# pacargile/ThePayne

Hardware: AMD Instinct MI355X
Metric: likelihood-evals/sec (4k-pixel ANN, 512 live points) (higher is better)
Workload: dtype f32; 1 GPU; C2: single star per GPU, 4096-pixel 2x300 YST1 ANN, 3600 observed pixels, batch of 512 candidate vectors per step (dynesty live points); batch=512, npix=4096, nobs=3600, stars=1, kernel_variant=0, parallelism=1 star per GPU, no data-path collective, products=2 x fp16 parts, 3 products, fp32 accumulator

## Files before the change

include/payne_hip.h:

```cpp
#ifndef PAYNE_HIP_H
#define PAYNE_HIP_H

#ifdef __cplusplus
extern "C" {
#endif

#define PAYNE_ABI_VERSION 2

#define PAYNE_OK 0
#define PAYNE_E_INVALID (-1)
#define PAYNE_E_UNSUPPORTED (-2)
#define PAYNE_E_HIP (-3)
#define PAYNE_E_BATCH (-4)
#define PAYNE_E_SIGMA (-5)

#define PAYNE_ACT_NONE 0
#define PAYNE_ACT_LRELU 1
#define PAYNE_ACT_SIGMOID 2

#define PAYNE_MAX_LAYERS 8
#define PAYNE_MAX_LABELS 5
#define PAYNE_MAX_POLY 12

typedef struct payne_layer {
// ... 44 lines not shown
} payne_opts;

#define PAYNE_V_OUT_GENERIC 1u
#define PAYNE_V_POST_GENERIC 2u
#define PAYNE_V_TW_GLOBAL 4u
#define PAYNE_V_POST_FULL 8u
#define PAYNE_V_NO_PREP 16u
#define PAYNE_V_SELECT_MEDIAN 64u
#define PAYNE_V_NO_WALK_TAIL 512u
#define PAYNE_V_OUT_BK64 1024u
#define PAYNE_V_OUT_ROLLED 2048u
#define PAYNE_V_OUT_F32 4096u
#define PAYNE_V_SED_OWN_LAUNCH 8192u
#define PAYNE_V_OUT_SMALL_TILES 16384u
#define PAYNE_V_BIG_WORKSPACE 65536u
#define PAYNE_V_NO_WALK_SPEC 131072u
#define PAYNE_V_ROWS_PIXEL 262144u
#define PAYNE_V_OUT_PLANES 524288u
#define PAYNE_V_OUT_BF16X3 1048576u
#define PAYNE_V_HID_F32 2097152u
#define PAYNE_V_HID_CHAIN 4194304u
#define PAYNE_V_HID_WAVES4 8388608u
#define PAYNE_V_OUT_WHOLE_TILE 16777216u
#define PAYNE_V_LSF_GLOBAL 128u

typedef struct payne_ctx payne_ctx;

int payne_version(void);

int payne_ctx_create(const payne_model_desc* model, const payne_obs_desc* obs,
                     const payne_phot_desc* phot, const payne_opts* opts, int device,
                     payne_ctx** out);

int payne_ctx_set_obs(payne_ctx* ctx, const payne_obs_desc* obs);

int payne_ctx_set_continuum(payne_ctx* ctx, const payne_model_desc* cont);

int payne_ctx_set_lsf(payne_ctx* ctx, const double* lsf, int n);
int payne_ctx_set_lsf_on(payne_ctx* ctx, const double* lsf_wave, const double* lsf, int n);

void payne_ctx_destroy(payne_ctx* ctx);

const char* payne_last_error(const payne_ctx* ctx);

int payne_theta_cols(const payne_ctx* ctx);

// ... 161 lines not shown
```

thepayne_amd/_lib.py:

```python
import ctypes as C
import os

HERE = os.path.dirname(os.path.abspath(__file__))
LIB_PATH = os.path.join(HERE, "libpayne_hip.so")

PAYNE_MAX_LAYERS = 8
PAYNE_MAX_POLY = 12
ACT_NONE, ACT_LRELU, ACT_SIGMOID = 0, 1, 2
F_FWHM_R = 1
SMOOTH_VEL_DIRECT, SMOOTH_WAVE_DIRECT, SMOOTH_LSF_DIRECT, SMOOTH_WAVE_FFT, SMOOTH_INTERP = range(5)
ABI_VERSION = 2
E_INVALID, E_UNSUPPORTED, E_HIP, E_BATCH, E_SIGMA = -1, -2, -3, -4, -5
V_OUT_GENERIC, V_POST_GENERIC, V_TW_GLOBAL, V_POST_FULL, V_NO_PREP, V_SELECT_MEDIAN, V_LSF_GLOBAL, V_NO_WALK_TAIL, V_OUT_BK64, V_OUT_ROLLED, V_OUT_F32, V_SED_OWN_LAUNCH, V_BIG_WORKSPACE = 1, 2, 4, 8, 16, 64, 128, 512, 1024, 2048, 4096, 8192, 65536
V_OUT_SMALL_TILES = 16384
V_NO_WALK_SPEC = 131072
V_ROWS_PIXEL = 262144
V_OUT_PLANES = 524288
V_OUT_BF16X3 = 1048576
V_HID_F32 = 2097152
V_HID_CHAIN = 4194304
V_HID_WAVES4 = 8388608
V_OUT_WHOLE_TILE = 16777216

SYMBOLS = ["payne_version", "payne_ctx_create", "payne_ctx_set_obs", "payne_ctx_set_continuum", "payne_ctx_set_lsf", "payne_ctx_set_lsf_on", "payne_ctx_destroy", "payne_last_error",
           "payne_theta_cols", "payne_lnlike_batch", "payne_predict_batch", "payne_smooth_batch", "payne_smooth_direct", "payne_sed_batch", "payne_bc_batch", "payne_kernel_name", "payne_last_kernel", "payne_activation_batch",
           "payne_profile", "payne_profile_read",
           "payne_sampler_create", "payne_sampler_destroy", "payne_prior_transform_batch", "payne_lnprob_u_batch",
           "payne_rwalk_batch", "payne_rwalk_begin", "payne_rwalk_begin_ell", "payne_rwalk_step", "payne_sampler_counters", "payne_ns_rwalk_queue", "payne_ns_rwalk_queue_begin", "payne_ns_rwalk_queue_end", "payne_ns_rwalk_queue_turn", "payne_ns_consume", "payne_ns_peek", "payne_ns_bound", "payne_format_rows",
           "payne_ns_queue_dev_init", "payne_ns_queue_dev_launch", "payne_ns_queue_dev_collect"]

PAYNE_MAX_DIM, PAYNE_MAX_FIXED = 24, 16
PRIOR_UNIFORM, PRIOR_GAUSSIAN, PRIOR_TGAUSSIAN, PRIOR_EXP, PRIOR_TEXP, PRIOR_LOGUNIFORM, PRIOR_TABLE = range(7)

_dp = C.POINTER(C.c_double)


class Layer(C.Structure):
    _fields_ = [("w", C.c_void_p), ("b", C.c_void_p), ("n_in", C.c_int), ("n_out", C.c_int), ("act", C.c_int)]


class ModelDesc(C.Structure):
    _fields_ = [("n_layers", C.c_int), ("layers", Layer * PAYNE_MAX_LAYERS), ("n_labels", C.c_int),
                ("xmin", _dp), ("xmax", _dp), ("npix", C.c_int), ("wavelength", _dp), ("resolution", C.c_double)]


# ... 171 lines not shown
```

thepayne_amd/csrc/k_post_full_a.hip:

```cpp
#define PAYNE_TU_POST_FULL_A
#include <hip/hip_runtime.h>

#include "../../include/payne_hip.h"
#include "post_seq.hpp"

using namespace payne;
#include "post_kernels.hpp"
PAYNE_POST_FULL_A_LIST(PAYNE_POST_DEFINE)
```

thepayne_amd/csrc/k_post_lean.hip:

```cpp
#define PAYNE_TU_POST_LEAN
#include <hip/hip_runtime.h>

#include "../../include/payne_hip.h"
#include "post_seq.hpp"

using namespace payne;
#include "post_kernels.hpp"
PAYNE_POST_LEAN_LIST(PAYNE_POST_DEFINE)
```

thepayne_amd/csrc/payne_hip.hip:

```cpp
#include <hip/hip_runtime.h>

#include <chrono>
#include <cstdio>
#include <cstdlib>
#include <cstring>
#include <string>
#include <thread>
#include <vector>

#include "../../include/payne_hip.h"
#include "host_tables.hpp"
#include "post_seq.hpp"
#include "ns_core.hpp"

using namespace payne;

#include "dense_kernels.hpp"

#include "post_kernels.hpp"

#include "sed_kernel.hpp"
#include "select.hpp"

__global__ void payne_photonly_kernel(const double* mags, const double* obs, const double* err, int F, int B, double* lnl) {
// ... 467 lines not shown
      }
      c->big_tiled = true;
      c->big_chip = T.n1 == kChipN1 && c->H.geo && !(opts->variant & PAYNE_V_BIG_WORKSPACE);
      if (c->big_chip) {
        he = hipFuncSetAttribute(reinterpret_cast<const void*>(payne_post_chip_kernel), hipFuncAttributeMaxDynamicSharedMemorySize,
                                 (int)kChipLdsBytes);
        if (he != hipSuccess) return bail(fail(c, PAYNE_E_HIP, std::string("hipFuncSetAttribute(chip): ") + hipGetErrorString(he)));
      }
      if (c->big_tiled) {
        he = hipFuncSetAttribute(reinterpret_cast<const void*>(payne_post_big_kernel), hipFuncAttributeMaxDynamicSharedMemorySize,
                                 (int)(2 * fft_tile_complex() * sizeof(c32)));
        if (he != hipSuccess) return bail(fail(c, PAYNE_E_HIP, std::string("hipFuncSetAttribute(big): ") + hipGetErrorString(he)));
      }
    }
    c->post_lds = (size_t)(T.n1 > 16384 ? 64 : fft_buf_floats(T.n1)) * 8 + (size_t)scratch_doubles(kPostThreads) * 8 + ((sizeof(CandState) + 15) & ~(size_t)15) + 16;
    const size_t tw_bytes = c->H.twf.size() * sizeof(c32);
    c->post_tw_lds = (c->post_lds + tw_bytes) <= 80 * 1024;
    if (opts->variant & PAYNE_V_TW_GLOBAL) c->post_tw_lds = false;
    if (c->post_tw_lds) c->post_lds += tw_bytes;
#ifdef PAYNE_STAMPS
    if (const char* e = getenv("PAYNE_DIAG_LDS")) c->post_lds = std::max(c->post_lds, (size_t)atoi(e));
#endif
    const int geom_n1 = (opts->variant & PAYNE_V_POST_GENERIC) ? 0 : T.n1;
    c->post_fn = pick_post_kernel(geom_n1, c->post_tw_lds);
    c->post_fn_lean = (opts->variant & PAYNE_V_POST_FULL) ? c->post_fn : pick_post_kernel(geom_n1, c->post_tw_lds, true);
    c->lean_available = c->post_fn_lean != c->post_fn;
    he = hipFuncSetAttribute(reinterpret_cast<const void*>(c->post_fn_lean), hipFuncAttributeMaxDynamicSharedMemorySize, (int)c->post_lds);
    if (he != hipSuccess) return bail(fail(c, PAYNE_E_HIP, std::string("hipFuncSetAttribute: ") + hipGetErrorString(he)));
    he = hipFuncSetAttribute(reinterpret_cast<const void*>(c->post_fn), hipFuncAttributeMaxDynamicSharedMemorySize, (int)c->post_lds);
    if (he != hipSuccess) return bail(fail(c, PAYNE_E_HIP, std::string("hipFuncSetAttribute: ") + hipGetErrorString(he)));
    {
      const bool fixed = geom_n1 != 0 && ((c->post_tw_lds && (T.n1 == 1024 || T.n1 == 2048 || T.n1 == 4096)) || (!c->post_tw_lds && T.n1 == 8192));
      const bool ident = T.rot_identity && T.n1 == model->npix;
      if (((fixed || c->big_chip || c->big_chip2) && ident || (fixed && !ident)) && c->w_out_p3 && c->hid_p3 && !(opts->variant & PAYNE_V_ROWS_PIXEL)) {
        const payne_layer& L = model->layers[model->n_layers - 1];
        const int K = L.n_in, Kp = c->w_out_kp, n = ident ? L.n_out : T.n1;
        std::vector<float> W((size_t)L.n_out * K), b((size_t)L.n_out), Wz, bz;
        he = hipMemcpy(W.data(), L.w, W.size() * 4, hipMemcpyDeviceToHost);
        if (he == hipSuccess) he = hipMemcpy(b.data(), L.b, b.size() * 4, hipMemcpyDeviceToHost);
        if (he != hipSuccess) return bail(fail(c, PAYNE_E_HIP, std::string("hipMemcpy(output layer): ") + hipGetErrorString(he)));
        if (ident) freq_rows(W.data(), b.data(), -(double)kBase, n, K, Wz, bz, c->big_chip ? 1 : (c->big_chip2 ? 2 : 0));
        else {
          freq_rows(W.data(), b.data(), -(double)kBase, n, K, Wz, bz, 0, c->H.rs1_idx.data(), c->H.rs1_frac.data(), L.n_out);
          c->freq_rs = true;
          if ((rc = dev_alloc(c, (size_t)1, &c->rot_flag, c->owned))) return bail(rc);
        }
        std::vector<float> Wp((size_t)n * Kp, 0.f);
        for (int i = 0; i < n; ++i) std::copy(Wz.begin() + (size_t)i * K, Wz.begin() + (size_t)(i + 1) * K, Wp.begin() + (size_t)i * Kp);
// ... 607 lines not shown
  a.prep = c->prep_valid ? c->prep : nullptr;
  const bool lean = stage < 0 && !out && a.prep && !c->big_ws;
  if (tail && lean && c->lean_available) {
    a.tail = tail->dev; a.tail_step = tail->step; a.tail_propose = tail->propose; tail->done = true;
    a.tail_spec = (c->spec_launched && tail->propose && tail->spec) ? 1 : 0;
  }
  {
    ProfScope ps(c, s, 1);
    if (c->big_ws && c->big_chip) {
      const int grid = B < c->big_grid ? B : c->big_grid;
      PAYNE_LAUNCH(payne_post_chip_kernel, dim3(grid), dim3(kChipThreads), kChipLdsBytes, s, c->T, a, c->big_ws, B);
    } else if (c->big_ws && c->big_chip2) {
      const int pairs = (B + 1) / 2, grid = pairs < c->big_grid ? pairs : c->big_grid;
      PAYNE_LAUNCH(payne_post_chip2_kernel, dim3(grid), dim3(kChipThreads), kChipLdsBytes, s, c->T, a, c->big_ws, B);
    } else if (c->big_ws) {
      const int grid = B < c->big_grid ? B : c->big_grid;
      const int tiled = c->big_tiled ? 1 : 0;
      const size_t lds = (tiled & 1) ? 2 * (size_t)fft_tile_complex() * sizeof(c32) : 0;
      PAYNE_LAUNCH(payne_post_big_kernel, dim3(grid), dim3(kBigThreads), lds, s, c->T, a, c->big_ws, B, tiled);
    } else {
      if (!post_lead_fits(a.ld_raw, a.ld_theta, a.n_filters)) return fail(c, PAYNE_E_INVALID, "row pitch / theta columns / filters beyond what the post kernel's packed arguments hold");
      PAYNE_LAUNCH(lean ? c->post_fn_lean : c->post_fn, dim3(B), dim3(kPostThreads), c->post_lds, s, c->T.twf, a.raw, a.prep, a.theta,
                   a.rot_flag, a.mags, post_lead_ints(a.ld_raw, a.ld_theta, a.n_filters, c->T.raw_freq), (unsigned)a.rot_seq, c->T, a);
      c->last_kernel[1] = post_kernel_label((c->opts.variant & PAYNE_V_POST_GENERIC) ? 0 : c->T.n1, c->post_tw_lds, lean && c->lean_available);
    }
  }
  hipError_t e = hipGetLastError();
  if (e != hipSuccess) return fail(c, PAYNE_E_HIP, std::string("post launch: ") + hipGetErrorString(e));
  return PAYNE_OK;
}

static int run_post_lsf(payne_ctx* c, const double* theta, int B, int stage, float* out, int ld_out, double* lnl,
                        bool with_phot, hipStream_t s) {
  const bool had = c->has_lsf;
  for (int off = 0; off < B; off += c->lsf_chunk) {
    const int nb = std::min(c->lsf_chunk, B - off);
    const double* th = theta + (size_t)off * c->ncols;
    c->has_lsf = false;
    const float* raw_all = c->raw;
    const CandState* prep_all = c->prep;
    c->raw = const_cast<float*>(raw_all) + (size_t)off * c->T.npix;
    c->prep = const_cast<CandState*>(prep_all) + off;
    int rc = run_post(c, th, nb, 1.0, 5, c->lsf_spec, c->T.npix, nullptr, false, s);
    c->raw = const_cast<float*>(raw_all); c->prep = const_cast<CandState*>(prep_all);
    c->has_lsf = had;
    if (rc) return rc;
    LsfArgs a{};
// ... 1026 lines not shown
```

thepayne_amd/csrc/post_core.hpp:

```cpp
#pragma once
#include <math.h>
#include <stdint.h>

#ifdef __HIPCC__
#define PAYNE_HD __host__ __device__ __forceinline__
#define PAYNE_HD_COLD __host__ __device__ inline __attribute__((noinline))
#else
#define PAYNE_HD inline
#define PAYNE_HD_COLD inline
#endif

namespace payne {

constexpr double kCkms = 2.998e5;
constexpr double kCDoppler = 299792.458;
constexpr double kPi = 3.141592653589793;
constexpr float kBase = 1.0f;
constexpr double kVsTabStep = 1.0 / 64.0;
constexpr double kVsTabMax = 256.0;
constexpr double kPosMagic = 1572864.0;
constexpr unsigned kPosMagicHi = 0x41380000u;
constexpr int kObsPad = 8192;
#ifndef PAYNE_POST_THREADS
#define PAYNE_POST_THREADS 512
// ... 506 lines not shown
        w[2] = ldc1(twf, OFF + P + k); w[4] = ldc1(twf, OFF + 2 * P + k);
        w[3] = cmul(w[1], w[2]); w[5] = cmul(w[1], w[4]); w[6] = cmul(w[2], w[4]); w[7] = cmul(w[3], w[4]);
      } else if constexpr (R == 4) {
        w[2] = cmul(w[1], w[1]); w[3] = cmul(w[2], w[1]);
      }
      twiddle_all<R>(u, w);
    }
    dftR<R>(u);
    const int j = fft_lay<PO, R>((i - k) * R + k);
#pragma unroll
    for (int r = 0; r < R; ++r) {
      c32 v = u[r];
      union { float f; unsigned b; } cv;
      cv.f = v.y; cv.b ^= sign; v.y = cv.f;
      if constexpr (last) {
        if (r == 0 && edge && i == 0) v.x = v.y;
        if (r == R - 1 && edge && i == NB - 1) v.y = v.x;
      }
      stc(dst, j + r * P, v);
    }
  }
}

PAYNE_HD_COLD double vsini_sb_exact(double ub) {
  double s, c;
#ifdef __HIP_DEVICE_COMPILE__
  sincos(ub, &s, &c);
#else
  s = sin(ub); c = cos(ub);
#endif
  double u2 = ub * ub;
  return j1(ub) / ub - 3.0 * c / (2.0 * u2) + 3.0 * s / (2.0 * (u2 * ub));
}
typedef float tap2 __attribute__((vector_size(8)));
struct TapPos { int i; float f; };
PAYNE_HD TapPos vsini_tab_pos(int tab_n, double vs_c64, int k, bool& far) {
  const double tm = fma((double)k, vs_c64, kPosMagic);
  const bool in = tm < kPosMagic + (double)(tab_n - 3);
  far = far || !in;
  union { double d; unsigned long long u; } cv;
  cv.d = in ? tm : kPosMagic;
  TapPos p;
  p.i = (int)((unsigned)(cv.u >> 32) & 0x7FFFFu);
  p.f = (float)(unsigned)cv.u * 2.3283064365386963e-10f;
  return p;
}
// ... 978 lines not shown
```

thepayne_amd/csrc/post_kernels.hpp:

```cpp
#pragma once
#include "select.hpp"
#include "sampler_core.hpp"
#include "post_onchip.hpp"
#include "post_onchip2.hpp"

constexpr int kStampRow = 192;
struct PostArgs {
  const double* theta; int ld_theta;
  double instr_factor;
  const float* raw; int ld_raw;
  float* out; int ld_out; int out_stage;
  double* lnl;
  const double* mags; int n_filters;
  const double* obs_mag; const double* obs_err;
  unsigned long long* stamps;
  int stamp_sparse;
  const CandState* prep;
  const WalkTail* tail; int tail_step, tail_propose;
  int tail_spec;
  const unsigned long long* rot_flag; unsigned long long rot_seq; int ld_raw_alt;
};

template <bool BUF_LDS, bool TW_LDS, int NTHR = 0>
struct DevExecT {
  static __device__ __forceinline__ int nthr_() { if constexpr (NTHR > 0) return NTHR; else return (int)blockDim.x; }
  static constexpr bool kTwLds = TW_LDS;
#ifdef __HIP_DEVICE_COMPILE__
  static __device__ __forceinline__ auto buf(c32* p) {
    if constexpr (BUF_LDS) return (PAYNE_AS_LDS f2v*)p; else return (PAYNE_AS_GLOBAL f2v*)p;
  }
  static __device__ __forceinline__ auto twid(const c32* p) {
    if constexpr (TW_LDS) return (const PAYNE_AS_LDS f2v*)p; else return (const PAYNE_AS_GLOBAL f2v*)p;
  }
  static __device__ __forceinline__ auto lds(c32* p) { return (PAYNE_AS_LDS f2v*)p; }
#else
  static c32* buf(c32* p) { return p; }
  static const c32* twid(const c32* p) { return p; }
  static c32* lds(c32* p) { return p; }
#endif
#ifdef PAYNE_STAMPS
  unsigned long long* stamps = nullptr;
  int nst = 0;
  bool sparse = false;
#endif
  template <class F>
  __device__ __forceinline__ void par(F&& f) {
// ... 11 lines not shown
#endif
  }
  __device__ __forceinline__ int nthreads() const { return nthr_(); }
  c32* tile_ = nullptr;
  __device__ __forceinline__ c32* tile() const { return tile_; }
};

__device__ __forceinline__ double sed_chi2(const double* mags, const double* obs, const double* err, int F) {
  double s = 0.0;
  for (int f = 0; f < F; ++f) { const double d = mags[f] - obs[f]; s += (d * d) / (err[f] * err[f]); }
  return s;
}

__device__ __attribute__((noinline)) static void walk_tail(const WalkTail* t, int b, int lane, double lnl, int step, int propose) {
  const WalkState W = uniform_copy(&t->w);
  rwalk_step_wave(t->sd, W, b, lane, lnl, step, 1, propose);
}

__device__ __attribute__((noinline)) static void walk_tail_spec(const WalkTail* t, int b, int lane, double lnl) {
  const WalkState W = uniform_copy(&t->w);
  rwalk_settle_spec(W, b, lane, lnl);
}

template <int LOG2N, bool TW_LDS, bool LEAN = false>
#if PAYNE_POST_THREADS > 512
#define PAYNE_POST_BOUNDS __launch_bounds__(kPostThreads) __attribute__((amdgpu_waves_per_eu(8, 8)))
#else
#define PAYNE_POST_BOUNDS __launch_bounds__(kPostThreads)
#endif
__global__ void PAYNE_POST_BOUNDS payne_post_kernel(const c32* lead_twf, const float* lead_raw, const CandState* lead_prep, const double* lead_theta, const unsigned long long* lead_rot_flag, const double* lead_mags, unsigned lead_ints, unsigned lead_rot_seq, const PostTables T_, PostArgs a_) {
  PostTables T = T_;
  T.twf = lead_twf; T.raw_freq = (int)(lead_ints >> 31);
  PostArgs a = a_;
  a.raw = lead_raw; a.prep = lead_prep; a.theta = lead_theta; a.rot_flag = lead_rot_flag; a.mags = lead_mags;
  a.ld_raw = (int)(lead_ints & 0x1ffffu); a.ld_theta = (int)((lead_ints >> 17) & 0x3fu); a.n_filters = (int)((lead_ints >> 23) & 0xffu);
  extern __shared__ __attribute__((aligned(16))) unsigned char smem[];
  const int n1 = LOG2N > 0 ? (1 << LOG2N) : T.n1;
  int raw_freq = T.raw_freq, ld_raw = a.ld_raw;
  if (a.rot_flag != nullptr && (unsigned)*a.rot_flag == lead_rot_seq) { raw_freq = 0; ld_raw = a.ld_raw_alt; }
  float* bufA = reinterpret_cast<float*>(smem);
  float* bufB = bufA + fft_buf_floats(n1);
  double* red = reinterpret_cast<double*>(bufB + fft_buf_floats(n1));
  CandState* S = reinterpret_cast<CandState*>(red + scratch_doubles(kPostThreads));
  const c32* twf = T.twf;
  typedef float f2g __attribute__((ext_vector_type(2)));
  constexpr int NTW = LOG2N > 0 ? plan_table_len((1 << (LOG2N > 0 ? LOG2N : 1)) / 2) : 1, PER = (NTW + kPostThreads - 1) / kPostThreads;
  f2g tw_tmp[PER];
  const int ntw_copy = (LOG2N > 0 && TW_LDS && raw_freq) ? plan_total((1 << (LOG2N > 0 ? LOG2N : 1)) / 2) : NTW;
  if (TW_LDS) {
    c32* twl = reinterpret_cast<c32*>(reinterpret_cast<unsigned char*>(S) + ((sizeof(CandState) + 15) & ~(size_t)15));
    const f2g* __restrict__ g = reinterpret_cast<const f2g*>(T.twf);
    f2g* tl = reinterpret_cast<f2g*>(twl);
    if constexpr (LOG2N > 0) {
// ... 14 lines not shown
  const bool sed_lane = sed_early && (int)threadIdx.x >= 64 && (int)threadIdx.x < 64 + a.n_filters;
  double sed_m = 0.0, sed_o = 0.0, sed_e = 1.0;
  if (sed_lane) {
    const int f = (int)threadIdx.x - 64;
    sed_m = a.mags[(size_t)b * a.n_filters + f]; sed_o = a.obs_mag[f]; sed_e = a.obs_err[f];
  }
  auto early = [&]() {
    if constexpr (TW_LDS && LOG2N > 0) {
      f2g* tl = reinterpret_cast<f2g*>(reinterpret_cast<unsigned char*>(S) + ((sizeof(CandState) + 15) & ~(size_t)15));
#pragma unroll
      for (int q = 0; q < PER; ++q) asm volatile("" : "+v"(tw_tmp[q]));
      const int ncopy = raw_freq ? plan_total((1 << (LOG2N > 0 ? LOG2N : 1)) / 2) : NTW;
#pragma unroll
      for (int q = 0; q < PER; ++q) {
        const int i0 = (int)threadIdx.x + q * kPostThreads;
        if (i0 < ncopy) tl[i0] = tw_tmp[q];
      }
    }
    if (a.mags != nullptr && a.n_filters <= 64 && (int)threadIdx.x >= 64 && (int)threadIdx.x < 64 + a.n_filters) {
      const double d = sed_m - sed_o;
      sed_terms[(int)threadIdx.x - 64] = (d * d) / (sed_e * sed_e);
    }
  };
  DevExecT<true, TW_LDS, kPostThreads> ex;
#ifdef PAYNE_STAMPS
  if (a.stamps) {
    ex.stamps = a.stamps + (size_t)b * kStampRow;
    if (threadIdx.x == 0) { ex.stamps[1] = __builtin_amdgcn_s_memtime(); }
    ex.nst = 1;
    ex.sparse = a.stamp_sparse != 0;
  }
#endif
  double* chi2 = red + scratch_doubles(kPostThreads) - 1;
  const int ostage = LEAN ? -1 : a.out_stage;
  float* outp = LEAN ? nullptr : (a.out ? a.out + (size_t)b * a.ld_out : nullptr);
  const CandState* prep = a.prep ? a.prep + b : nullptr;
  if (LEAN) { prep = a.prep + b; __builtin_assume(prep != nullptr); }
  run_candidate<LOG2N, kPostThreads>(ex, T, twf, a.theta + (size_t)b * a.ld_theta, a.instr_factor,
                                     a.raw + (size_t)b * ld_raw, bufA, bufB, *S, red, outp, ostage, chi2, prep, early, raw_freq);
  double lnl_v = 0.0;
  if (threadIdx.x == 0 && a.lnl && ostage < 0) {
    double x2 = *chi2;
    if (sed_early) { double sx = 0.0; for (int f = 0; f < a.n_filters; ++f) sx += sed_terms[f]; x2 += sx; }
    else if (a.mags) x2 += sed_chi2(a.mags + (size_t)b * a.n_filters, a.obs_mag, a.obs_err, a.n_filters);
    lnl_v = -0.5 * x2;
    a.lnl[b] = lnl_v;
  }
  if constexpr (LEAN) {
    if (a.tail && threadIdx.x < 64) {
      const double l = __shfl(lnl_v, 0);
      if (a.tail_spec) walk_tail_spec(a.tail, b, (int)threadIdx.x, l);
      else walk_tail(a.tail, b, (int)threadIdx.x, l, a.tail_step, a.tail_propose);
    }
  }
#ifdef PAYNE_STAMPS
  if (a.stamps && threadIdx.x == 0) { ex.stamps[0] = (unsigned long long)ex.nst; ex.stamps[kStampRow - 1] = __builtin_amdgcn_s_memtime(); }
#endif
}


#ifndef PAYNE_BIG_THREADS
#define PAYNE_BIG_THREADS 512
#endif
constexpr int kBigThreads = PAYNE_BIG_THREADS;
#ifndef PAYNE_TU_BIG
__global__ void __launch_bounds__(kBigThreads) payne_post_big_kernel(const PostTables T, PostArgs a, float* ws, int B, int tile_lds);
#else
__global__ void __launch_bounds__(kBigThreads) payne_post_big_kernel(const PostTables T, PostArgs a, float* ws, int B, int tile_lds) {
  __shared__ double red[kBigThreads + kBigThreads / 2 + 2];
  __shared__ CandState S;
  extern __shared__ __attribute__((aligned(16))) unsigned char big_sm[];
  float* bufA = ws + (size_t)blockIdx.x * 2 * T.n1;
  float* bufB = bufA + T.n1;
  DevExecT<false, false> ex;
  if (tile_lds & 1) ex.tile_ = reinterpret_cast<c32*>(big_sm);
  double* chi2 = red + scratch_doubles(kBigThreads) - 1;
  for (int b = blockIdx.x; b < B; b += gridDim.x) {
#ifdef PAYNE_STAMPS
    if (a.stamps) {
      ex.stamps = a.stamps + (size_t)b * kStampRow;
      if (threadIdx.x == 0) ex.stamps[1] = __builtin_amdgcn_s_memtime();
      ex.nst = 1;
    }
#endif
    run_candidate<0, kBigThreads>(ex, T, T.tw, a.theta + (size_t)b * a.ld_theta, a.instr_factor,
                                  a.raw + (size_t)b * a.ld_raw, bufA, bufB, S, red,
                                  a.out ? a.out + (size_t)b * a.ld_out : nullptr, a.out_stage, chi2,
                                  a.prep ? a.prep + b : nullptr);
    if (threadIdx.x == 0 && a.lnl && a.out_stage < 0) {
      double x2 = *chi2;
      if (a.mags) x2 += sed_chi2(a.mags + (size_t)b * a.n_filters, a.obs_mag, a.obs_err, a.n_filters);
      a.lnl[b] = -0.5 * x2;
    }
#ifdef PAYNE_STAMPS
    if (a.stamps && threadIdx.x == 0) ex.stamps[0] = (unsigned long long)ex.nst;
#endif
    __syncthreads();
  }
}

#endif

namespace payne { template <bool TW, int N> struct ex_lds_tail<DevExecT<true, TW, N>> { static constexpr bool value = true; }; }
struct ChipExec : DevExecT<false, false> {
#ifdef __HIP_DEVICE_COMPILE__
  ChipLds L;
#endif
};
namespace payne { template <> struct ex_chip<ChipExec> { static constexpr bool value = true; }; }
#ifdef __HIP_DEVICE_COMPILE__
namespace payne {
template <bool VSINI, class Ex>
PAYNE_SEQ float* chip_conv_stage(Ex& ex, float* work, const TaperArgs& ta, bool& edge, const float* src0, const Window* rs, bool zin, bool scrub) {
  if constexpr (ex_chip<Ex>::value) {
    if (rs) {
      __shared__ ChipResample R;
      if (threadIdx.x == 0) R = chip_resample_of(*rs);
      __syncthreads();
      chip_conv<VSINI>(ex.L, src0, work, ta, false, edge, (int)threadIdx.x, &R, false);
    } else {
      chip_conv<VSINI>(ex.L, src0 ? src0 : work, work, ta, src0 != nullptr && scrub, edge, (int)threadIdx.x, nullptr, zin && src0 != nullptr);
    }
    ex.mark(0);
    edge = false;
  }
  return work;
// ... 435 lines not shown
    __syncthreads();
    red[tid] = accx;
    __syncthreads();
    if (tid == 0) {
      double x2 = 0.0;
      for (int t = 0; t < 256; ++t) x2 += red[t];
      if (a.mags) x2 += sed_chi2(a.mags + (size_t)b * a.n_filters, a.obs_mag, a.obs_err, a.n_filters);
      a.lnl[b] = -0.5 * x2;
    }
  }
}

template __global__ void payne_lsf_kernel<false>(const PostTables, LsfArgs);
template __global__ void payne_lsf_kernel<true>(const PostTables, LsfArgs);
#else
template <bool GLOBAL> __global__ void payne_lsf_kernel(const PostTables T, LsfArgs a);
extern template __global__ void payne_lsf_kernel<false>(const PostTables, LsfArgs);
extern template __global__ void payne_lsf_kernel<true>(const PostTables, LsfArgs);
#endif

#define PAYNE_POST_LEAN_LIST(X) X(12, true, true) X(11, true, true) X(10, true, true) X(13, false, true)
#define PAYNE_POST_FULL_A_LIST(X) X(12, true, false) X(0, true, false)
#define PAYNE_POST_FULL_B_LIST(X) X(10, true, false) X(11, true, false) X(13, false, false) X(0, false, false)
#define PAYNE_POST_SIG const c32*, const float*, const CandState*, const double*, const unsigned long long*, const double*, unsigned, unsigned, const PostTables, PostArgs
static inline bool post_lead_fits(int ld_raw, int ld_theta, int n_filters) { return ld_raw >= 0 && ld_raw < (1 << 17) && ld_theta >= 0 && ld_theta < 64 && n_filters >= 0 && n_filters < 256; }
static inline unsigned post_lead_ints(int ld_raw, int ld_theta, int n_filters, int raw_freq) {
  return (unsigned)ld_raw | ((unsigned)ld_theta << 17) | ((unsigned)n_filters << 23) | ((unsigned)(raw_freq != 0) << 31);
}
#define PAYNE_POST_EXTERN(L, TW, LEAN) extern template __global__ void payne_post_kernel<L, TW, LEAN>(PAYNE_POST_SIG);
#define PAYNE_POST_DEFINE(L, TW, LEAN) template __global__ void payne_post_kernel<L, TW, LEAN>(PAYNE_POST_SIG);
#ifndef PAYNE_TU_POST_LEAN
PAYNE_POST_LEAN_LIST(PAYNE_POST_EXTERN)
#endif
#ifndef PAYNE_TU_POST_FULL_A
PAYNE_POST_FULL_A_LIST(PAYNE_POST_EXTERN)
#endif
#ifndef PAYNE_TU_POST_FULL_B
PAYNE_POST_FULL_B_LIST(PAYNE_POST_EXTERN)
#endif

typedef void (*post_kernel_fn)(PAYNE_POST_SIG);
static const char* post_kernel_label(int n1, bool tw_lds, bool lean) {
  if (lean) {
    if (tw_lds && n1 == 4096) return "payne_post_kernel<12, true, true>";
    if (tw_lds && n1 == 2048) return "payne_post_kernel<11, true, true>";
    if (tw_lds && n1 == 1024) return "payne_post_kernel<10, true, true>";
    if (!tw_lds && n1 == 8192) return "payne_post_kernel<13, false, true>";
  }
  if (tw_lds) return n1 == 1024 ? "payne_post_kernel<10, true>" : n1 == 2048 ? "payne_post_kernel<11, true>" : n1 == 4096 ? "payne_post_kernel<12, true>" : "payne_post_kernel<0, true>";
  return n1 == 8192 ? "payne_post_kernel<13, false>" : "payne_post_kernel<0, false>";
}
static post_kernel_fn pick_post_kernel(int n1, bool tw_lds, bool lean = false) {
  if (lean) {
    if (tw_lds && n1 == 4096) return payne_post_kernel<12, true, true>;
    if (tw_lds && n1 == 2048) return payne_post_kernel<11, true, true>;
    if (tw_lds && n1 == 1024) return payne_post_kernel<10, true, true>;
    if (!tw_lds && n1 == 8192) return payne_post_kernel<13, false, true>;
  }
  if (tw_lds) {
    switch (n1) {
      case 1024: return payne_post_kernel<10, true>;
      case 2048: return payne_post_kernel<11, true>;
      case 4096: return payne_post_kernel<12, true>;
      default: return payne_post_kernel<0, true>;
    }
  }
  switch (n1) {
    case 8192: return payne_post_kernel<13, false>;
    default: return payne_post_kernel<0, false>;
  }
}
```

thepayne_amd/csrc/post_seq.hpp:

```cpp
#pragma once
#include "post_core.hpp"

#ifdef __HIPCC__
#define PAYNE_SEQ __device__ __forceinline__
#define PAYNE_SEQ_CALL __device__ __attribute__((noinline))
#else
#define PAYNE_SEQ inline
#define PAYNE_SEQ_CALL inline
#endif

namespace payne {

PAYNE_HD int scratch_doubles(int nthr) { return nthr + nthr / 2 + 2; }

template <class Ex>
PAYNE_SEQ c32* fft_run_tiled(Ex& ex, c32* a_, c32* b_, int M, const c32* tw_, int tw_n, bool conj_last, c32* tile);
template <class Ex>
PAYNE_SEQ c32* fft_run(Ex& ex, c32* a, c32* b, int M, const c32* tw, int tw_n, bool conj_last) {
  if (c32* tile = ex.tile())
    if (fft_tiled_ok(M)) return fft_run_tiled(ex, a, b, M, tw, tw_n, conj_last, tile);
  c32 *src = a, *dst = b;
  int p = 1;
  while (p < M) {
    const int R = pass_radix(M, p);
// ... 46 lines not shown
  return a_;
}

template <int M, int P, int NT, class Ex, class BP, class TP>
PAYNE_SEQ BP fft_fixed_passes(Ex& ex, BP src, BP dst, TP twf, unsigned sign_last, bool edge) {
  if constexpr (P >= M) {
    return src;
  } else {
    constexpr int R = plan_radix(M, P);
    constexpr bool last = (P * R >= M);
    const unsigned sign = last ? sign_last : 0u;
    ex.par([&](int t, int) { fft_pass_fixed<R, M, P, NT>(t, src, dst, twf, sign, last && edge); });
    return fft_fixed_passes<M, P * R, NT>(ex, dst, src, twf, sign_last, edge);
  }
}
template <int M, int NT, class Ex>
PAYNE_SEQ_CALL c32* fft_fixed(Ex& ex, c32* src, c32* dst, const c32* twf, unsigned sign_last, bool edge) {
  auto s = Ex::buf(src);
  auto d = Ex::buf(dst);
  return fft_fixed_passes<M, 1, NT>(ex, s, d, Ex::twid(twf), sign_last, edge) == s ? src : dst;
}

template <class Ex> struct ex_lds_tail { static constexpr bool value = false; };
#ifdef __HIP_DEVICE_COMPILE__
__device__ __forceinline__ void post_lds_barrier() { asm volatile("s_waitcnt lgkmcnt(0)\n\ts_barrier" ::: "memory"); }
template <int M, int P, int NT, class BP, class TP>
__device__ __forceinline__ BP fft_fixed_passes_lds(int tid, BP src, BP dst, TP twf, unsigned sign_last) {
  if constexpr (P >= M) {
    return src;
  } else {
    constexpr int R = plan_radix(M, P);
    constexpr bool last = (P * R >= M);
    fft_pass_fixed<R, M, P, NT>(tid, src, dst, twf, last ? sign_last : 0u, false);
    post_lds_barrier();
    return fft_fixed_passes_lds<M, P * R, NT>(tid, dst, src, twf, sign_last);
  }
}
template <int M, int NT, int OU, class Ex>
__device__ __forceinline__ double inverse_and_obs(int tid, const PostTables& T, const CandState& S, const Window& W, const c32* twf,
                                                  c32* z, c32* zo) {
  ObsRec rec[OU];
  obs_fast_issue<OU>(NT, T, tid, rec);
  auto r = fft_fixed_passes_lds<M, 1, NT>(tid, Ex::buf(z), Ex::buf(zo), Ex::twid(twf), 0x80000000u);
  const float* conv = (r == Ex::buf(z)) ? (const float*)z : (const float*)zo;
  return phase_obs<OU>(tid, NT, T, S, W, conv, nullptr, -1, false, &rec);
}
#endif

constexpr int kChipN1 = 65536;
template <class Ex> struct ex_chip { static constexpr bool value = false; };
template <bool VSINI, class Ex>
PAYNE_SEQ float* chip_conv_stage(Ex& ex, float* work, const TaperArgs& ta, bool& edge, const float* src0, const Window* rs, bool zin, bool scrub);

template <int LOG2N, int NT, bool VSINI, class Ex>
PAYNE_SEQ float* conv_stage(Ex& ex, const PostTables& T, const c32* twf, float* work, float* other, int n,
                            const TaperArgs& ta, bool& edge, const float* src0 = nullptr, const Window* rs = nullptr,
                            bool have_y = false,
                            bool zin = false, bool scrub = true,
                            bool defer_inverse = false) {
  const int M = n / 2;
  if constexpr (ex_chip<Ex>::value) {
    if (n == kChipN1) return chip_conv_stage<VSINI>(ex, work, ta, edge, src0, rs, zin, scrub);
  }
  if constexpr (LOG2N > 0) {
    constexpr int MF = (1 << LOG2N) / 2;
    if (M == MF) {
      c32* z = have_y ? (c32*)work : fft_fixed<MF, NT>(ex, (c32*)work, (c32*)other, twf, 0u, false);
      constexpr int PU = unroll_for((1 << LOG2N) / NT) / 4;
      if (!have_y) ex.par([&](int t, int) { rfft_taper_phase<VSINI, PU>(t, NT, Ex::buf(z), MF, Ex::twid(twf + plan_total(MF)), 1, ta); });
      c32* zo = ((float*)z == work) ? (c32*)other : (c32*)work;
      if (defer_inverse) return (float*)z;
      float* res = (float*)fft_fixed<MF, NT>(ex, z, zo, twf, 0x80000000u, edge);
      edge = false;
      return res;
    }
  }
  const c32* tw = T.tw;
  c32* z = fft_run(ex, (c32*)work, (c32*)other, M, tw, T.nmax, false);
  ex.par([&](int t, int nt) { rfft_taper_phase<VSINI>(t, nt, z, M, tw, T.nmax / (2 * M), ta); });
  c32* zo = ((float*)z == work) ? (c32*)other : (c32*)work;
  return (float*)fft_run(ex, z, zo, M, tw, T.nmax, true);
}

struct NoEarly { PAYNE_HD void operator()() const {} };
template <int LOG2N, int NT, class Ex, class Early = NoEarly>
PAYNE_SEQ void run_candidate(Ex& ex, const PostTables& T, const c32* twf, const double* th, double instr_factor,
                             const float* raw, float* bufA, float* bufB, CandState& S, double* red,
                             float* out, int out_stage, double* chi2_out, const CandState* prep = nullptr, Early early = Early(),
                             int raw_freq = -1) {
  const bool rawf = raw_freq < 0 ? T.raw_freq != 0 : raw_freq != 0;
  const bool maybe_direct = (out_stage != 0) && T.rot_identity;
  const bool freq_chip = ex_chip<Ex>::value && T.n1 == kChipN1 && rawf;
  const bool freq = (LOG2N > 0 && rawf) || freq_chip;
  constexpr int MFq = LOG2N > 0 ? (1 << LOG2N) / 2 : 4;
  constexpr int SU = (MFq / 2 + NT - 1) / NT;
// ... 134 lines not shown
```

Baseline: 18.41 million likelihood-evals/s.

## Use wave-local radix-8 FFT passes for 2048-point post stage

Replaces the fixed 2048-point complex FFT in the post kernel with a schedule where four waves each run three radix-8 passes on a 512-point subsequence without block barriers, followed by one block-wide radix-4 cross pass. The default kernel now uses this wave-local path, and the old multi-barrier path is kept as a new opt-in four-pass variant. The intent is to cut block-wide LDS barriers per FFT. In exchange, only half the threads are busy during the local passes, and the padded block layout (576 stride) uses more LDS.

After: 18.49 million likelihood-evals/s, median of 6. About the same (+0.4%).

```diff
diff --git a/include/payne_hip.h b/include/payne_hip.h
--- a/include/payne_hip.h
+++ b/include/payne_hip.h
@@ -90,6 +90,7 @@
 #define PAYNE_V_HID_CHAIN 4194304u
 #define PAYNE_V_HID_WAVES4 8388608u
 #define PAYNE_V_OUT_WHOLE_TILE 16777216u
+#define PAYNE_V_POST_FOUR_PASS 33554432u
 #define PAYNE_V_LSF_GLOBAL 128u
 
 typedef struct payne_ctx payne_ctx;
diff --git a/thepayne_amd/_lib.py b/thepayne_amd/_lib.py
--- a/thepayne_amd/_lib.py
+++ b/thepayne_amd/_lib.py
@@ -21,6 +21,7 @@
 V_HID_CHAIN = 4194304
 V_HID_WAVES4 = 8388608
 V_OUT_WHOLE_TILE = 16777216
+V_POST_FOUR_PASS = 33554432
 
 SYMBOLS = ["payne_version", "payne_ctx_create", "payne_ctx_set_obs", "payne_ctx_set_continuum", "payne_ctx_set_lsf", "payne_ctx_set_lsf_on", "payne_ctx_destroy", "payne_last_error",
            "payne_theta_cols", "payne_lnlike_batch", "payne_predict_batch", "payne_smooth_batch", "payne_smooth_direct", "payne_sed_batch", "payne_bc_batch", "payne_kernel_name", "payne_last_kernel", "payne_activation_batch",
diff --git a/thepayne_amd/csrc/k_post_full_a.hip b/thepayne_amd/csrc/k_post_full_a.hip
--- a/thepayne_amd/csrc/k_post_full_a.hip
+++ b/thepayne_amd/csrc/k_post_full_a.hip
@@ -7,3 +7,4 @@
 using namespace payne;
 #include "post_kernels.hpp"
 PAYNE_POST_FULL_A_LIST(PAYNE_POST_DEFINE)
+PAYNE_POST_4P_FULL_LIST(PAYNE_POST_4P_DEFINE)
diff --git a/thepayne_amd/csrc/k_post_lean.hip b/thepayne_amd/csrc/k_post_lean.hip
--- a/thepayne_amd/csrc/k_post_lean.hip
+++ b/thepayne_amd/csrc/k_post_lean.hip
@@ -7,3 +7,4 @@
 using namespace payne;
 #include "post_kernels.hpp"
 PAYNE_POST_LEAN_LIST(PAYNE_POST_DEFINE)
+PAYNE_POST_4P_LEAN_LIST(PAYNE_POST_4P_DEFINE)
diff --git a/thepayne_amd/csrc/payne_hip.hip b/thepayne_amd/csrc/payne_hip.hip
--- a/thepayne_amd/csrc/payne_hip.hip
+++ b/thepayne_amd/csrc/payne_hip.hip
@@ -513,8 +513,9 @@
     if (const char* e = getenv("PAYNE_DIAG_LDS")) c->post_lds = std::max(c->post_lds, (size_t)atoi(e));
 #endif
     const int geom_n1 = (opts->variant & PAYNE_V_POST_GENERIC) ? 0 : T.n1;
-    c->post_fn = pick_post_kernel(geom_n1, c->post_tw_lds);
-    c->post_fn_lean = (opts->variant & PAYNE_V_POST_FULL) ? c->post_fn : pick_post_kernel(geom_n1, c->post_tw_lds, true);
+    const bool four_pass = (opts->variant & PAYNE_V_POST_FOUR_PASS) != 0;
+    c->post_fn = pick_post_kernel(geom_n1, c->post_tw_lds, false, four_pass);
+    c->post_fn_lean = (opts->variant & PAYNE_V_POST_FULL) ? c->post_fn : pick_post_kernel(geom_n1, c->post_tw_lds, true, four_pass);
     c->lean_available = c->post_fn_lean != c->post_fn;
     he = hipFuncSetAttribute(reinterpret_cast<const void*>(c->post_fn_lean), hipFuncAttributeMaxDynamicSharedMemorySize, (int)c->post_lds);
     if (he != hipSuccess) return bail(fail(c, PAYNE_E_HIP, std::string("hipFuncSetAttribute: ") + hipGetErrorString(he)));
@@ -1168,7 +1169,8 @@
       if (!post_lead_fits(a.ld_raw, a.ld_theta, a.n_filters)) return fail(c, PAYNE_E_INVALID, "row pitch / theta columns / filters beyond what the post kernel's packed arguments hold");
       PAYNE_LAUNCH(lean ? c->post_fn_lean : c->post_fn, dim3(B), dim3(kPostThreads), c->post_lds, s, c->T.twf, a.raw, a.prep, a.theta,
                    a.rot_flag, a.mags, post_lead_ints(a.ld_raw, a.ld_theta, a.n_filters, c->T.raw_freq), (unsigned)a.rot_seq, c->T, a);
-      c->last_kernel[1] = post_kernel_label((c->opts.variant & PAYNE_V_POST_GENERIC) ? 0 : c->T.n1, c->post_tw_lds, lean && c->lean_available);
+      c->last_kernel[1] = post_kernel_label((c->opts.variant & PAYNE_V_POST_GENERIC) ? 0 : c->T.n1, c->post_tw_lds, lean && c->lean_available,
+                                              (c->opts.variant & PAYNE_V_POST_FOUR_PASS) != 0);
     }
   }
   hipError_t e = hipGetLastError();
diff --git a/thepayne_amd/csrc/post_core.hpp b/thepayne_amd/csrc/post_core.hpp
--- a/thepayne_amd/csrc/post_core.hpp
+++ b/thepayne_amd/csrc/post_core.hpp
@@ -552,6 +552,57 @@
   }
 }
 
+#ifdef __HIP_DEVICE_COMPILE__
+constexpr int kWlM = 2048, kWlBlk = 576;
+template <int P, class SP, class DP, class TP>
+__device__ __forceinline__ void fft_pass_local8(int w, int lane, SP src, DP dst, TP twf) {
+  constexpr int R = 8, NB = 64, OFF = plan_offset(kWlM, P);
+  constexpr int PI = (P == 1) ? 0 : (P == 8 ? 1 : 8), RI = (P == 1) ? 0 : 8;
+  constexpr int PO = (P == 64) ? 0 : P;
+  static_assert(P == 1 || P == 8 || P == 64, "the three radix-8 passes");
+  int i = lane;
+  if constexpr (P == 1) i = (lane & ~31) | ((lane & 14) << 1) | ((lane >> 3) & 2) | (lane & 1);
+  const int k = i & (P - 1);
+  c32 u[R];
+  if constexpr (P == 1) {
+#pragma unroll
+    for (int r = 0; r < R; ++r) u[r] = ldc1(src, w + 4 * (i + r * NB));
+  } else {
+    const int ib = fft_lay<PI, RI>(i);
+#pragma unroll
+    for (int r = 0; r < R; ++r) u[r] = ldc1(src, ib + fft_lay<PI, RI>(r * NB));
+    c32 tw[R];
+    tw[1] = ldc1(twf, OFF + k); tw[2] = ldc1(twf, OFF + P + k); tw[4] = ldc1(twf, OFF + 2 * P + k);
+    tw[3] = cmul(tw[1], tw[2]); tw[5] = cmul(tw[1], tw[4]); tw[6] = cmul(tw[2], tw[4]); tw[7] = cmul(tw[3], tw[4]);
+    twiddle_all<R>(u, tw);
+  }
+  dftR<R>(u);
+  const int j = fft_lay<PO, R>((i - k) * R + k);
+#pragma unroll
+  for (int r = 0; r < R; ++r) stc(dst, j + r * P, u[r]);
+}
+template <class SP, class DP, class TP>
+__device__ __forceinline__ void fft_pass_cross4(int i, SP src, DP dst, TP twf, unsigned sign, bool edge) {
+  constexpr int R = 4, NB = kWlM / R, OFF = plan_offset(kWlM, NB);
+  c32 u[R];
+#pragma unroll
+  for (int r = 0; r < R; ++r) u[r] = ldc1(src, i + r * kWlBlk);
+  c32 tw[R];
+  tw[1] = ldc1(twf, OFF + i); tw[2] = cmul(tw[1], tw[1]); tw[3] = cmul(tw[2], tw[1]);
+  twiddle_all<R>(u, tw);
+  dftR<R>(u);
+#pragma unroll
+  for (int r = 0; r < R; ++r) {
+    c32 v = u[r];
+    union { float f; unsigned b; } cv;
+    cv.f = v.y; cv.b ^= sign; v.y = cv.f;
+    if (r == 0 && edge && i == 0) v.x = v.y;
+    if (r == R - 1 && edge && i == NB - 1) v.y = v.x;
+    stc(dst, i + r * NB, v);
+  }
+}
+#endif
+
 PAYNE_HD_COLD double vsini_sb_exact(double ub) {
   double s, c;
 #ifdef __HIP_DEVICE_COMPILE__
diff --git a/thepayne_amd/csrc/post_kernels.hpp b/thepayne_amd/csrc/post_kernels.hpp
--- a/thepayne_amd/csrc/post_kernels.hpp
+++ b/thepayne_amd/csrc/post_kernels.hpp
@@ -21,7 +21,7 @@
   const unsigned long long* rot_flag; unsigned long long rot_seq; int ld_raw_alt;
 };
 
-template <bool BUF_LDS, bool TW_LDS, int NTHR = 0>
+template <bool BUF_LDS, bool TW_LDS, int NTHR = 0, bool WAVE_LOCAL = false>
 struct DevExecT {
   static __device__ __forceinline__ int nthr_() { if constexpr (NTHR > 0) return NTHR; else return (int)blockDim.x; }
   static constexpr bool kTwLds = TW_LDS;
@@ -79,13 +79,13 @@
   rwalk_settle_spec(W, b, lane, lnl);
 }
 
-template <int LOG2N, bool TW_LDS, bool LEAN = false>
 #if PAYNE_POST_THREADS > 512
 #define PAYNE_POST_BOUNDS __launch_bounds__(kPostThreads) __attribute__((amdgpu_waves_per_eu(8, 8)))
 #else
 #define PAYNE_POST_BOUNDS __launch_bounds__(kPostThreads)
 #endif
-__global__ void PAYNE_POST_BOUNDS payne_post_kernel(const c32* lead_twf, const float* lead_raw, const CandState* lead_prep, const double* lead_theta, const unsigned long long* lead_rot_flag, const double* lead_mags, unsigned lead_ints, unsigned lead_rot_seq, const PostTables T_, PostArgs a_) {
+template <int LOG2N, bool TW_LDS, bool LEAN, bool WAVE_LOCAL>
+__device__ __forceinline__ void post_kernel_body(const c32* lead_twf, const float* lead_raw, const CandState* lead_prep, const double* lead_theta, const unsigned long long* lead_rot_flag, const double* lead_mags, unsigned lead_ints, unsigned lead_rot_seq, const PostTables& T_, const PostArgs& a_) {
   PostTables T = T_;
   T.twf = lead_twf; T.raw_freq = (int)(lead_ints >> 31);
   PostArgs a = a_;
@@ -146,7 +146,7 @@
       sed_terms[(int)threadIdx.x - 64] = (d * d) / (sed_e * sed_e);
     }
   };
-  DevExecT<true, TW_LDS, kPostThreads> ex;
+  DevExecT<true, TW_LDS, kPostThreads, WAVE_LOCAL> ex;
 #ifdef PAYNE_STAMPS
   if (a.stamps) {
     ex.stamps = a.stamps + (size_t)b * kStampRow;
@@ -181,6 +181,14 @@
   if (a.stamps && threadIdx.x == 0) { ex.stamps[0] = (unsigned long long)ex.nst; ex.stamps[kStampRow - 1] = __builtin_amdgcn_s_memtime(); }
 #endif
 }
+template <int LOG2N, bool TW_LDS, bool LEAN = false>
+__global__ void PAYNE_POST_BOUNDS payne_post_kernel(const c32* lead_twf, const float* lead_raw, const CandState* lead_prep, const double* lead_theta, const unsigned long long* lead_rot_flag, const double* lead_mags, unsigned lead_ints, unsigned lead_rot_seq, const PostTables T_, PostArgs a_) {
+  post_kernel_body<LOG2N, TW_LDS, LEAN, true>(lead_twf, lead_raw, lead_prep, lead_theta, lead_rot_flag, lead_mags, lead_ints, lead_rot_seq, T_, a_);
+}
+template <int LOG2N, bool TW_LDS, bool LEAN = false>
+__global__ void PAYNE_POST_BOUNDS payne_post_kernel_4p(const c32* lead_twf, const float* lead_raw, const CandState* lead_prep, const double* lead_theta, const unsigned long long* lead_rot_flag, const double* lead_mags, unsigned lead_ints, unsigned lead_rot_seq, const PostTables T_, PostArgs a_) {
+  post_kernel_body<LOG2N, TW_LDS, LEAN, false>(lead_twf, lead_raw, lead_prep, lead_theta, lead_rot_flag, lead_mags, lead_ints, lead_rot_seq, T_, a_);
+}
 
 
 #ifndef PAYNE_BIG_THREADS
@@ -225,7 +233,10 @@
 
 #endif
 
-namespace payne { template <bool TW, int N> struct ex_lds_tail<DevExecT<true, TW, N>> { static constexpr bool value = true; }; }
+namespace payne {
+template <bool TW, int N, bool WL> struct ex_lds_tail<DevExecT<true, TW, N, WL>> { static constexpr bool value = true; };
+template <bool TW> struct ex_wave_local<DevExecT<true, TW, 512, true>> { static constexpr bool value = true; };
+}
 struct ChipExec : DevExecT<false, false> {
 #ifdef __HIP_DEVICE_COMPILE__
   ChipLds L;
@@ -707,6 +718,8 @@
 #define PAYNE_POST_LEAN_LIST(X) X(12, true, true) X(11, true, true) X(10, true, true) X(13, false, true)
 #define PAYNE_POST_FULL_A_LIST(X) X(12, true, false) X(0, true, false)
 #define PAYNE_POST_FULL_B_LIST(X) X(10, true, false) X(11, true, false) X(13, false, false) X(0, false, false)
+#define PAYNE_POST_4P_LEAN_LIST(X) X(12, true, true)
+#define PAYNE_POST_4P_FULL_LIST(X) X(12, true, false)
 #define PAYNE_POST_SIG const c32*, const float*, const CandState*, const double*, const unsigned long long*, const double*, unsigned, unsigned, const PostTables, PostArgs
 static inline bool post_lead_fits(int ld_raw, int ld_theta, int n_filters) { return ld_raw >= 0 && ld_raw < (1 << 17) && ld_theta >= 0 && ld_theta < 64 && n_filters >= 0 && n_filters < 256; }
 static inline unsigned post_lead_ints(int ld_raw, int ld_theta, int n_filters, int raw_freq) {
@@ -714,18 +727,23 @@
 }
 #define PAYNE_POST_EXTERN(L, TW, LEAN) extern template __global__ void payne_post_kernel<L, TW, LEAN>(PAYNE_POST_SIG);
 #define PAYNE_POST_DEFINE(L, TW, LEAN) template __global__ void payne_post_kernel<L, TW, LEAN>(PAYNE_POST_SIG);
+#define PAYNE_POST_4P_EXTERN(L, TW, LEAN) extern template __global__ void payne_post_kernel_4p<L, TW, LEAN>(PAYNE_POST_SIG);
+#define PAYNE_POST_4P_DEFINE(L, TW, LEAN) template __global__ void payne_post_kernel_4p<L, TW, LEAN>(PAYNE_POST_SIG);
 #ifndef PAYNE_TU_POST_LEAN
 PAYNE_POST_LEAN_LIST(PAYNE_POST_EXTERN)
+PAYNE_POST_4P_LEAN_LIST(PAYNE_POST_4P_EXTERN)
 #endif
 #ifndef PAYNE_TU_POST_FULL_A
 PAYNE_POST_FULL_A_LIST(PAYNE_POST_EXTERN)
+PAYNE_POST_4P_FULL_LIST(PAYNE_POST_4P_EXTERN)
 #endif
 #ifndef PAYNE_TU_POST_FULL_B
 PAYNE_POST_FULL_B_LIST(PAYNE_POST_EXTERN)
 #endif
 
 typedef void (*post_kernel_fn)(PAYNE_POST_SIG);
-static const char* post_kernel_label(int n1, bool tw_lds, bool lean) {
+static const char* post_kernel_label(int n1, bool tw_lds, bool lean, bool four_pass = false) {
+  if (four_pass && tw_lds && n1 == 4096) return lean ? "payne_post_kernel_4p<12, true, true>" : "payne_post_kernel_4p<12, true>";
   if (lean) {
     if (tw_lds && n1 == 4096) return "payne_post_kernel<12, true, true>";
     if (tw_lds && n1 == 2048) return "payne_post_kernel<11, true, true>";
@@ -735,7 +753,8 @@
   if (tw_lds) return n1 == 1024 ? "payne_post_kernel<10, true>" : n1 == 2048 ? "payne_post_kernel<11, true>" : n1 == 4096 ? "payne_post_kernel<12, true>" : "payne_post_kernel<0, true>";
   return n1 == 8192 ? "payne_post_kernel<13, false>" : "payne_post_kernel<0, false>";
 }
-static post_kernel_fn pick_post_kernel(int n1, bool tw_lds, bool lean = false) {
+static post_kernel_fn pick_post_kernel(int n1, bool tw_lds, bool lean = false, bool four_pass = false) {
+  if (four_pass && tw_lds && n1 == 4096) return lean ? payne_post_kernel_4p<12, true, true> : payne_post_kernel_4p<12, true, false>;
   if (lean) {
     if (tw_lds && n1 == 4096) return payne_post_kernel<12, true, true>;
     if (tw_lds && n1 == 2048) return payne_post_kernel<11, true, true>;
diff --git a/thepayne_amd/csrc/post_seq.hpp b/thepayne_amd/csrc/post_seq.hpp
--- a/thepayne_amd/csrc/post_seq.hpp
+++ b/thepayne_amd/csrc/post_seq.hpp
@@ -92,8 +92,24 @@
 }
 
 template <class Ex> struct ex_lds_tail { static constexpr bool value = false; };
+template <class Ex> struct ex_wave_local { static constexpr bool value = false; };
 #ifdef __HIP_DEVICE_COMPILE__
 __device__ __forceinline__ void post_lds_barrier() { asm volatile("s_waitcnt lgkmcnt(0)\n\ts_barrier" ::: "memory"); }
+template <int NT, class BP, class TP>
+__device__ __forceinline__ BP fft_wave_local(int tid, BP src, BP dst, TP twf, unsigned sign_last, bool edge) {
+  static_assert(NT == 512, "four waves own a 512-point subsequence each, eight run the radix-4 pass");
+  if (tid < 256) {
+    const int w = tid >> 6, l = tid & 63;
+    auto blk = dst + kWlBlk * w;
+    fft_pass_local8<1>(w, l, src, blk, twf);
+    fft_pass_local8<8>(w, l, blk, blk, twf);
+    fft_pass_local8<64>(w, l, blk, blk, twf);
+  }
+  post_lds_barrier();
+  fft_pass_cross4(tid, dst, src, twf, sign_last, edge);
+  post_lds_barrier();
+  return src;
+}
 template <int M, int P, int NT, class BP, class TP>
 __device__ __forceinline__ BP fft_fixed_passes_lds(int tid, BP src, BP dst, TP twf, unsigned sign_last) {
   if constexpr (P >= M) {
@@ -111,11 +127,31 @@
                                                   c32* z, c32* zo) {
   ObsRec rec[OU];
   obs_fast_issue<OU>(NT, T, tid, rec);
-  auto r = fft_fixed_passes_lds<M, 1, NT>(tid, Ex::buf(z), Ex::buf(zo), Ex::twid(twf), 0x80000000u);
+  auto r = Ex::buf(z);
+#ifdef PAYNE_EXP_NO_FFT2K
+  if constexpr (M == kWlM) {} else
+#endif
+  if constexpr (ex_wave_local<Ex>::value && M == kWlM) r = fft_wave_local<NT>(tid, Ex::buf(z), Ex::buf(zo), Ex::twid(twf), 0x80000000u, false);
+  else r = fft_fixed_passes_lds<M, 1, NT>(tid, Ex::buf(z), Ex::buf(zo), Ex::twid(twf), 0x80000000u);
   const float* conv = (r == Ex::buf(z)) ? (const float*)z : (const float*)zo;
   return phase_obs<OU>(tid, NT, T, S, W, conv, nullptr, -1, false, &rec);
 }
 #endif
+
+template <int M, int NT, class Ex>
+PAYNE_SEQ c32* fft_fixed_stage(Ex& ex, c32* src, c32* dst, const c32* twf, unsigned sign_last, bool edge) {
+#ifdef PAYNE_EXP_NO_FFT2K
+  if constexpr (M == 2048) return src;
+#endif
+#ifdef __HIP_DEVICE_COMPILE__
+  if constexpr (ex_wave_local<Ex>::value && M == kWlM) {
+    fft_wave_local<NT>((int)threadIdx.x, Ex::buf(src), Ex::buf(dst), Ex::twid(twf), sign_last, edge);
+    ex.mark(0);
+    return src;
+  }
+#endif
+  return fft_fixed<M, NT>(ex, src, dst, twf, sign_last, edge);
+}
 
 constexpr int kChipN1 = 65536;
 template <class Ex> struct ex_chip { static constexpr bool value = false; };
@@ -135,12 +171,12 @@
   if constexpr (LOG2N > 0) {
     constexpr int MF = (1 << LOG2N) / 2;
     if (M == MF) {
-      c32* z = have_y ? (c32*)work : fft_fixed<MF, NT>(ex, (c32*)work, (c32*)other, twf, 0u, false);
+      c32* z = have_y ? (c32*)work : fft_fixed_stage<MF, NT>(ex, (c32*)work, (c32*)other, twf, 0u, false);
       constexpr int PU = unroll_for((1 << LOG2N) / NT) / 4;
       if (!have_y) ex.par([&](int t, int) { rfft_taper_phase<VSINI, PU>(t, NT, Ex::buf(z), MF, Ex::twid(twf + plan_total(MF)), 1, ta); });
       c32* zo = ((float*)z == work) ? (c32*)other : (c32*)work;
       if (defer_inverse) return (float*)z;
-      float* res = (float*)fft_fixed<MF, NT>(ex, z, zo, twf, 0x80000000u, edge);
+      float* res = (float*)fft_fixed_stage<MF, NT>(ex, z, zo, twf, 0x80000000u, edge);
       edge = false;
       return res;
     }
```
